# cvg/nicer-slam

Hardware: AMD Instinct MI355X
Metric: rays/sec (fwd+bwd), one tracking iteration (higher is better)
Workload: dtype f32; 1 GPU; Replica room0 tracking iteration, 1024 rays x 128 samples (+640 sampler evaluations/ray), single MI355X, fp32 [BASELINE configs[1]]; rays_per_gpu=1024, samples_per_ray=128, sampler_evals_per_ray=640, global_rays=1024, engine=fused, param_grads=False, hip_graph=True, driver=KernelTracker, python_gc=off inside the timed regions (as timeit), ray_chunks=1, cache_prewarm_steps=100, cache_prewarm_batches=disjoint from the warm-up and timed batches, parallelism=single, rccl_ranks=0, full=False

## Files before the change

nicer_slam_amd/csrc/colour_fwd_body.inc:

```
    desync_simd_partners();
    const int lane = threadIdx.x & 63;
    const int h = lane >> 5;
    const uint32_t tile = blockIdx.x * 4 + (threadIdx.x >> 6);
    if (tile * 32 >= a.src.P) return;
    const bool wave_live = true;
    uint32_t pid = tile * 32 + (lane & 31);
    const bool live = pid < a.src.P;
    if (!live) pid = a.src.P - 1;
    const uint32_t q = point_of(a.src, pid);
    float x[3], z, dir[3];
    uint32_t ray;
    load_point(a.src, q, x, ray, z);
#pragma unroll
    for (int d = 0; d < 3; ++d) dir[d] = a.src.rays_d[ray * 3 + d];
    float in[COL_IN_STEPS];
    colour_inputs(a, geom, tile, q, lane, h, x, dir, in, false, wave_live);
    f32x16 a1[2], a2[2];
    float rgb[3];
    uint32_t masks[2] = {0u, 0u};
    colour_mlp<Seq, false>(nullptr, a.wp, lane, h, in, a1, a2, rgb, a.save ? masks : nullptr);
    if (live && h == 0) {
#pragma unroll
        for (int j = 0; j < 3; ++j) a.rgb[(size_t)q * 3 + j] = rgb[j];
    }
    if (a.save) {
        float* ext = save_ext(a.save, a.src.P, tile);
        ext[lane] = __uint_as_float(masks[0]);
        ext[64 + lane] = __uint_as_float(masks[1]);
        if (h == 0) {
#pragma unroll
            for (int j = 0; j < 3; ++j) ext[128 + 32 * j + (lane & 31)] = rgb[j];
        }
    }
```

nicer_slam_amd/csrc/render_colour.hip:

```cpp
#include <cstdlib>
#include "sdf_net.hpp"

namespace nsa {

constexpr int CL = 16, CC = 2;

struct ColPack {
    static constexpr int kHH = a_block_floats(2, HS);
    static constexpr int kW0 = 0;
    static constexpr int kB0 = kW0 + a_block_floats(2, COL_IN_STEPS);
    static constexpr int kW1 = kB0 + 64;
    static constexpr int kB1 = kW1 + kHH;
    static constexpr int kW2V = kB1 + 64;
    static constexpr int kB2 = kW2V + 3 * 64;
    static constexpr int kW1T = kB2 + 64;
    static constexpr int kW0T = kW1T + kHH;
    static constexpr int kTotal = kW0T + a_block_floats(5, HS);
};

constexpr int kColStage = 7680;
template <bool BWD>
struct ColOps {
    static constexpr int n = BWD ? 6 : 3;
    __host__ __device__ static constexpr StageOp op(int i) {
        return i == 0 ? StageOp{ColPack::kW0, 2, 9, 0, 5} : i == 1 ? StageOp{ColPack::kW0, 2, 9, 5, 4}
             : i == 2 ? StageOp{ColPack::kW1, 2, 4, 0, 4} : i == 3 ? StageOp{ColPack::kW1T, 2, 4, 0, 4}
             : i == 4 ? StageOp{ColPack::kW0T, 5, 4, 0, 2} : StageOp{ColPack::kW0T, 5, 4, 2, 2};
    }
};

template <bool MAP>
struct ColBwdOps {
    static constexpr int n = MAP ? 6 : 3;
    static constexpr int kRev = MAP ? 3 : 0;
    __host__ __device__ static constexpr StageOp op(int i) { return ColOps<true>::op(MAP ? i : i + 3); }
};

constexpr int kSaveTile = 4096, kSaveExt = 256;
__device__ __forceinline__ float* save_ext(float* save, uint32_t P, uint32_t tile) {
    return save + (size_t)((P + 31) / 32) * kSaveTile + (size_t)tile * kSaveExt;
}

__device__ __forceinline__ uint32_t relu_mask(const f32x16 (&a)[2]) {
    uint32_t m = 0;
#pragma unroll
    for (int t = 0; t < 2; ++t)
#pragma unroll
        for (int r = 0; r < 16; ++r) m |= a[t][r] > 0.0f ? (1u << (16 * t + r)) : 0u;
    return m;
}

struct ColourArgs {
    PointSrc src;
    const float* table;
    const float* wp;
    float divide_factor;
    const float* grad;
    const float* feat;
    float* rgb;
    float* save;
    int save_no_features;
    const float* g_rgb;
    float* g_feat;
    float* g_grad;
    float* g_x;
    float* g_dir;
    int grid_grad;
    float* g_table;
    float* emit;
    uint32_t emit_ld;
};

enum : int { CE_IN = 0, CE_H1 = 130, CE_H2 = 194, CE_AB1 = 258, CE_AB2 = 322, CE_OB = 386, CE_ROWS = 389 };

struct ColEmitter {
    float* base;
    uint32_t ld;
    bool live;
    __device__ __forceinline__ void slot(int region, int s, int h, float v) const {
        base[(size_t)(region + 2 * s + h) * ld] = live ? v : 0.0f;
    }
    __device__ __forceinline__ void hid(int region, int q, int h, float v) const {
        const int f = 32 * (q >> 4) + (q & 3) + 8 * ((q & 15) >> 2) + 4 * h;
        base[(size_t)(region + f) * ld] = live ? v : 0.0f;
    }
};

__device__ __forceinline__ void colour_level_out(const float (&v)[8][CC], const float (&w)[3], const float (&dw)[3], float scale,
                                                 bool inside, int jl, float (&in)[COL_IN_STEPS], float* sv, bool sv_features = true) {
    float f[CC];
    blend<3, CC>(v, w, f);
#pragma unroll
    for (int c = 0; c < CC; ++c) in[49 + jl * CC + c] = inside ? f[c] : 0.0f;
    if (sv) {
        if (sv_features) {
#pragma unroll
            for (int c = 0; c < CC; ++c) sv[(jl * CC + c) * 64] = in[49 + jl * CC + c];
        }
#pragma unroll
        for (int gd = 0; gd < 3; ++gd) {
            float jr[CC];
            jacobian_row<3, CC>(v, w, dw, scale, gd, jr);
#pragma unroll
            for (int c = 0; c < CC; ++c) sv[(16 + (jl * 3 + gd) * CC + c) * 64] = inside ? jr[c] : 0.0f;
        }
    }
}

__device__ __forceinline__ void colour_inputs(const ColourArgs& a, const GridGeom16& geom, uint32_t tile, uint32_t q, int lane,
                                              int h, const float (&x)[3], const float (&dir)[3], float (&in)[COL_IN_STEPS],
                                              bool from_save, bool wave_live) {
    const float* fsrc = a.feat + (size_t)tile * 32 * 64 + lane;
#pragma unroll
    for (int q = 0; q < HS; ++q) in[q] = fsrc[q * 64];
    float gr[3];
#pragma unroll
    for (int d = 0; d < 3; ++d) gr[d] = a.grad[(size_t)q * 3 + d];
    in[32] = h ? x[1] : x[0];
    in[33] = h ? dir[0] : x[2];
    in[34] = h ? dir[2] : dir[1];
    in[35] = h ? gr[1] : gr[0];
    in[36] = h ? 0.0f : gr[2];
#pragma unroll
    for (int j = 0; j < 6; ++j) {
        const int g0 = 2 * j, g1 = 2 * j + 1;
        const float da = h ? dir[g1 % 3] : dir[g0 % 3];
        const float sc = h ? (float)(1 << (g1 / 3)) : (float)(1 << (g0 / 3));
        sincos_f(da * sc, in[37 + 2 * j], in[38 + 2 * j]);
    }
    if (from_save) {
        const float* sv = a.save + (size_t)tile * 64 * 64 + lane;
#pragma unroll
        for (int q = 0; q < 16; ++q) in[49 + q] = sv[q * 64];
        return;
    }
    float u[3];
#pragma unroll
    for (int d = 0; d < 3; ++d) u[d] = to_unit(x[d], a.divide_factor);
    float* sv = (a.save && wave_live) ? a.save + (size_t)tile * 64 * 64 + lane : nullptr;
#pragma unroll
    for (int jl = 0; jl < CL / 2; ++jl) {
        const LevelGeom lg = geom.lv[2 * jl + h];
        uint32_t cell[3];
        float w[3], dw[3];
        const bool inside = locate<3>(u, lg.scale, cell, w, dw);
        float v[8][CC];
        gather_corners<3, CC>(a.table, lg, cell, v);
        colour_level_out(v, w, dw, lg.scale, inside, jl, in, sv, !a.save_no_features);
    }
}

template <class Seq, bool STAGED>
__device__ __forceinline__ void colour_mlp(float* stage, const float* __restrict__ wp, int lane, int h,
                                           const float (&in)[COL_IN_STEPS], f32x16 (&a1)[2], f32x16 (&a2)[2], float (&rgb)[3],
                                           uint32_t* masks = nullptr) {
    load_vec<2>(wp + ColPack::kB0, h, a1);
    if (STAGED) {
        const float m_in = abs_max<COL_IN_STEPS>(in);
        gemm_staged_part<Seq, kColStage, COL_IN_STEPS, 2, 0, 5, true, false>(stage, wp, 0, lane, in, a1, &m_in);
        gemm_staged_part<Seq, kColStage, COL_IN_STEPS, 2, 5, 4, false, true>(stage, wp, 1, lane, in, a1, &m_in);
    } else {
        gemm_op<COL_IN_STEPS, 2>(wp + ColPack::kW0, lane, in, a1);
    }
    const float m_h1 = acc_abs_max<2>(a1);
    float h1[HS];
#pragma unroll
    for (int t = 0; t < 2; ++t)
#pragma unroll
        for (int r = 0; r < 16; ++r) h1[16 * t + r] = relu_f(a1[t][r]);
    if (masks) masks[0] = relu_mask(a1);
    load_vec<2>(wp + ColPack::kB1, h, a2);
    if (STAGED) gemm_staged_part<Seq, kColStage, HS, 2, 0, 4>(stage, wp, 2, lane, h1, a2, &m_h1);
    else        gemm_op<HS, 2>(wp + ColPack::kW1, lane, h1, a2, &m_h1);
    if (masks) masks[1] = relu_mask(a2);
#pragma unroll
    for (int j = 0; j < 3; ++j) {
        f32x16 wv[2];
        load_vec<2>(wp + ColPack::kW2V + 64 * j, h, wv);
        float part = 0.0f;
#pragma unroll
        for (int t = 0; t < 2; ++t)
#pragma unroll
            for (int r = 0; r < 16; ++r) part = fmaf(relu_f(a2[t][r]), wv[t][r], part);
        const float o = xhalf_sum(part) + wp[ColPack::kB2 + j];
        rgb[j] = 1.0f / (1.0f + expf(-o));
    }
}

#ifndef NSA_OCC_COL_FWD
#define NSA_OCC_COL_FWD 4
#endif
__global__ __launch_bounds__(256, NSA_OCC_COL_FWD) void k_colour_fwd(ColourArgs a, GridGeom16 geom) {
    using Seq = ColOps<false>;
#include "colour_fwd_body.inc"
}

#ifdef NSA_X_TS
static __device__ unsigned long long* g_ts_c = nullptr;
#define CTS_BEGIN const unsigned long long ts_start = ts_now(); unsigned long long ts_prev = ts_start; \
    if ((threadIdx.x & 63) == 0) for (int i = 0; i < 16; ++i) nsa_ts_lds[threadIdx.x >> 6][i] = 0;
#define CTS_MARK(slot) { const unsigned long long t_ = ts_now(); ts_add(slot, t_ - ts_prev); ts_prev = t_; }
#define CTS_END { ts_add(15, ts_now() - ts_start); if (g_ts_c && (threadIdx.x & 63) == 0) { \
    unsigned long long* o_ = g_ts_c + ((size_t)blockIdx.x * (blockDim.x >> 6) + (threadIdx.x >> 6)) * 16; \
    for (int i = 0; i < 16; ++i) o_[i] = nsa_ts_lds[threadIdx.x >> 6][i]; } }
#else
#define CTS_BEGIN
#define CTS_MARK(slot)
#define CTS_END
#endif
template <bool MAP>
__global__ __launch_bounds__(256, 2) void k_colour_bwd(ColourArgs a, GridGeom16 geom) {
    using Seq = ColBwdOps<MAP>;
    __shared__ __attribute__((aligned(16))) float stage[2 * kColStage];
    CTS_BEGIN
#define NSA_BODY_NW 4
#include "colour_bwd_body.inc"
#undef NSA_BODY_NW
    CTS_MARK(11)
    CTS_END
}

}

#define NSA_SDFNET_AS_HEADER
#include "render_sdfnet.hip"
#undef NSA_SDFNET_AS_HEADER

namespace nsa {

#define NSA_CC_NW 4
#define NSA_BODY_NW NSA_CC_NW
__global__ __launch_bounds__(64 * NSA_CC_NW, 2) void k_colour_coarse_bwd(ColourArgs ca, GridGeom16 cgeom, SdfNetArgs sa, GridGeom16 sgeom) {
    __shared__ __attribute__((aligned(16))) float stage[2 * kStageFloats];
    static_assert(kStageFloats >= kColStage, "the colour phase stages its parts in the SDF kernel's buffers");
    float ho_fb[HS], ho_n[3], ho_gx[3];
#define NSA_BODY_HANDOFF
    {
        constexpr bool MAP = false;
        using Seq = ColBwdOps<false>;
        const ColourArgs& a = ca;
        const GridGeom16& geom = cgeom;
#include "colour_bwd_body.inc"
    }
    __syncthreads();
    {
        constexpr int L = 4, C = 8, NH = 1;
        constexpr bool MAP = false;
        using P = SdfPack<NH>;
        using Seq = SdfOps<NH, true>;
        const SdfNetArgs& a = sa;
        const GridGeom16& geom = sgeom;
#include "sdfnet_bwd_body.inc"
    }
#undef NSA_BODY_HANDOFF
}
#undef NSA_BODY_NW

}

#define NSA_COMPOSITE_AS_HEADER
#include "render_composite.hip"
#undef NSA_COMPOSITE_AS_HEADER

namespace nsa {

__global__ __launch_bounds__(256, NSA_OCC_COL_FWD) void k_colour_fwd_track(ColourArgs ca, GridGeom16 cgeom, CompositeArgs ta,
                                                                            const float* __restrict__ gt, float* __restrict__ ray_loss,
                                                                            float inv_n) {
    {
        using Seq = ColOps<false>;
        const ColourArgs& a = ca;
        const GridGeom16& geom = cgeom;
#include "colour_fwd_body.inc"
    }
    __syncthreads();
    if ((threadIdx.x >> 6) == 0) {
        const CompositeArgs& a = ta;
        const int lane = threadIdx.x & 63;
        const uint32_t ray = blockIdx.x;
#include "composite_track_body.inc"
    }
}

__global__ __launch_bounds__(256, NSA_OCC_COL_FWD) void k_colour_fwd_composite(ColourArgs ca, GridGeom16 cgeom, CompositeArgs ta) {
    {
        using Seq = ColOps<false>;
        const ColourArgs& a = ca;
        const GridGeom16& geom = cgeom;
#include "colour_fwd_body.inc"
    }
    __syncthreads();
    if ((threadIdx.x >> 6) == 0) {
        const CompositeArgs& a = ta;
        const int lane = threadIdx.x & 63;
        const uint32_t ray = blockIdx.x;
#include "composite_fwd_body.inc"
    }
}

}

#if defined(NSA_X_TS) && NSA_PIECES != 1
extern "C" int nsa_debug_set_ts_colour(unsigned long long* p) {
    return hipMemcpyToSymbol(HIP_SYMBOL(nsa::g_ts_c), &p, sizeof(p)) == hipSuccess ? 0 : 3;
}
#endif

#ifndef NSA_ENTRY
#define NSA_ENTRY(x) x
#endif
#include "bf16_entries.hpp"

extern "C" {

static int colour_common(const nsa_points_t* pts, const nsa_grid_t* grid, nsa::ColourArgs* a, nsa::GridGeom16* geom) {
    using namespace nsa;
    if (!pts || !grid) return NSA_EBADARG;
    if (pts->points || !pts->rays_o || !pts->rays_d || !pts->z_vals || pts->S == 0) return NSA_EBADARG;
    if (!(grid->L == 16 && grid->C == 2)) return NSA_EUNSUPPORTED_NET;
    if (int rc = make_grid_geom16(grid->offsets_host, grid->L, grid->S, grid->H, geom, grid->C)) return rc;
    a->src = PointSrc{pts->rays_o, pts->rays_d, pts->z_vals, nullptr, pts->P, pts->S, pts->order};
    a->table = grid->table;
    a->divide_factor = grid->divide_factor;
    return NSA_OK;
}

int NSA_ENTRY(nsa_colour_forward)(const nsa_points_t* pts, const nsa_grid_t* grid, const float* packed, const float* grad,
                       const float* feat_hl, float* rgb, float* save, nsa_stream_t stream) {
#if NSA_PIECES != 1
    if (grid && grid->precision == 1) return nsa_colour_forward_bf16(pts, grid, packed, grad, feat_hl, rgb, save, stream);
#endif
    using namespace nsa;
    if (!packed || !grad || !feat_hl || !rgb) return NSA_EBADARG;
    ColourArgs a{};
    GridGeom16 geom;
    if (int rc = colour_common(pts, grid, &a, &geom)) return rc;
    if (pts->P == 0) return NSA_OK;
    a.wp = packed; a.grad = grad; a.feat = feat_hl; a.rgb = rgb; a.save = save;
    const uint32_t tiles = (pts->P + 31) / 32;
    launch_begin();
    hipLaunchKernelGGL(k_colour_fwd, dim3((tiles + 3) / 4), dim3(256), 0, (hipStream_t)stream, a, geom);
    return launch_end();
}

int NSA_ENTRY(nsa_colour_forward_composite)(const nsa_points_t* pts, const nsa_grid_t* grid, const float* packed, const float* grad,
                                 const float* feat_hl, float* rgb, float* save, const float* sdf, const float* voxels,
                                 uint32_t voxel_res, float* weights, float* rgb_values, float* depth, float* nmap, float* entropy,
                                 nsa_stream_t stream) {
#if NSA_PIECES != 1
    if (grid && grid->precision == 1)
        return nsa_colour_forward_composite_bf16(pts, grid, packed, grad, feat_hl, rgb, save, sdf, voxels, voxel_res, weights, rgb_values,
                                                 depth, nmap, entropy, stream);
#endif
    using namespace nsa;
    if (!packed || !grad || !feat_hl || !rgb || !sdf || !voxels || !weights || !rgb_values || !depth || !nmap || !entropy)
        return NSA_EBADARG;
    ColourArgs a{};
    GridGeom16 geom;
    if (int rc = colour_common(pts, grid, &a, &geom)) return rc;
    if (pts->P == 0) return NSA_OK;
    if (pts->points || pts->order || pts->S != 128 || pts->P % 128 != 0) return NSA_EBADARG;
    a.wp = packed; a.grad = grad; a.feat = feat_hl; a.rgb = rgb; a.save = save;
    CompositeArgs t{};
    t.rays_o = pts->rays_o; t.rays_d = pts->rays_d; t.z_vals = pts->z_vals; t.sdf = sdf; t.rgb = rgb; t.grad = grad; t.voxels = voxels;
    t.voxel_res = voxel_res; t.R = pts->P / 128; t.S = 128;
    t.weights = weights; t.rgb_values = rgb_values; t.depth = depth; t.nmap = nmap; t.entropy = entropy;
    launch_begin();
    hipLaunchKernelGGL(k_colour_fwd_composite, dim3(pts->P / 128), dim3(256), 0, (hipStream_t)stream, a, geom, t);
    return launch_end();
}

int NSA_ENTRY(nsa_colour_forward_track)(const nsa_points_t* pts, const nsa_grid_t* grid, const float* packed, const float* grad,
                             const float* feat_hl, float* rgb, float* save, const float* sdf, const float* voxels, uint32_t voxel_res,
                             const float* gt, uint32_t n_total, float* rgb_values, float* ray_loss, float* g_sdf, float* g_rgb,
                             float* g_grad, nsa_stream_t stream) {
#if NSA_PIECES != 1
    if (grid && grid->precision == 1)
        return nsa_colour_forward_track_bf16(pts, grid, packed, grad, feat_hl, rgb, save, sdf, voxels, voxel_res, gt, n_total, rgb_values,
                                             ray_loss, g_sdf, g_rgb, g_grad, stream);
#endif
    using namespace nsa;
    if (!packed || !grad || !feat_hl || !rgb || !sdf || !voxels || !gt || !rgb_values || !ray_loss || !g_sdf || !g_rgb || !g_grad)
        return NSA_EBADARG;
    ColourArgs a{};
    GridGeom16 geom;
    if (int rc = colour_common(pts, grid, &a, &geom)) return rc;
    if (pts->P == 0) return NSA_OK;
    if (pts->points || pts->order || pts->S != 128 || pts->P % 128 != 0 || n_total < pts->P / 128) return NSA_EBADARG;
    a.wp = packed; a.grad = grad; a.feat = feat_hl; a.rgb = rgb; a.save = save;
#ifndef NSA_X_SAVE_FEATURES
    a.save_no_features = 1;
#endif
    CompositeArgs t{};
    t.rays_o = pts->rays_o; t.rays_d = pts->rays_d; t.z_vals = pts->z_vals; t.sdf = sdf; t.rgb = rgb; t.voxels = voxels;
    t.voxel_res = voxel_res; t.R = pts->P / 128; t.S = 128;
    t.rgb_values = rgb_values; t.g_sdf = g_sdf; t.g_rgb = g_rgb; t.g_grad = g_grad;
    launch_begin();
    hipLaunchKernelGGL(k_colour_fwd_track, dim3(pts->P / 128), dim3(256), 0, (hipStream_t)stream, a, geom, t, gt, ray_loss,
                       1.0f / (float)(3 * (uint64_t)n_total));
    return launch_end();
}

int NSA_ENTRY(nsa_colour_backward)(const nsa_points_t* pts, const nsa_grid_t* grid, const float* packed, const float* grad,
                        const float* feat_hl, const float* save, const float* g_rgb, int grid_grad, float* g_feat_hl,
                        float* g_grad, float* g_x, float* g_dir, nsa_stream_t stream) {
#if NSA_PIECES != 1
    if (grid && grid->precision == 1) return nsa_colour_backward_bf16(pts, grid, packed, grad, feat_hl, save, g_rgb, grid_grad, g_feat_hl, g_grad, g_x, g_dir, stream);
#endif
    using namespace nsa;
    if (!packed || !grad || !feat_hl || !save || !g_rgb || !g_feat_hl || !g_grad || !g_x || !g_dir) return NSA_EBADARG;
    ColourArgs a{};
    GridGeom16 geom;
    if (int rc = colour_common(pts, grid, &a, &geom)) return rc;
    if (pts->P == 0) return NSA_OK;
    a.wp = packed; a.grad = grad; a.feat = feat_hl; a.save = const_cast<float*>(save); a.g_rgb = g_rgb;
    a.g_feat = g_feat_hl; a.g_grad = g_grad; a.g_x = g_x; a.g_dir = g_dir; a.grid_grad = grid_grad;
    const uint32_t tiles = (pts->P + 31) / 32;
    launch_begin();
    hipLaunchKernelGGL(k_colour_bwd<false>, dim3((tiles + 3) / 4), dim3(256), 0, (hipStream_t)stream, a, geom);
    return launch_end();
}

int NSA_ENTRY(nsa_colour_coarse_backward)(const nsa_points_t* pts, const nsa_grid_t* grid, const float* packed, const float* grad,
                               const float* feat_hl, const float* save, const float* g_rgb, int grid_grad, float* g_feat_hl,
                               float* g_grad, float* g_x, float* g_dir, const nsa_grid_t* coarse, const float* packed_coarse,
                               const float* g_sdf, nsa_stream_t stream) {
#if NSA_PIECES != 1
    if (grid && coarse && grid->precision == 1 && coarse->precision == 1)
        return nsa_colour_coarse_backward_bf16(pts, grid, packed, grad, feat_hl, save, g_rgb, grid_grad, g_feat_hl, g_grad, g_x, g_dir, coarse,
                                               packed_coarse, g_sdf, stream);
#endif
    using namespace nsa;
    if (!packed || !grad || !feat_hl || !save || !g_rgb || !g_feat_hl || !g_grad || !g_x || !g_dir || !coarse || !packed_coarse)
        return NSA_EBADARG;
    if (grid->precision != coarse->precision) return NSA_EBADARG;
    if (coarse->tile == 16 || !(coarse->L == 4 && coarse->C == 8 && coarse->n_hidden == 1)) return NSA_EUNSUPPORTED_NET;
    ColourArgs a{};
    GridGeom16 geom, sgeom;
    if (int rc = colour_common(pts, grid, &a, &geom)) return rc;
    if (pts->P == 0) return NSA_OK;
    if (int rc = make_grid_geom16(coarse->offsets_host, coarse->L, coarse->S, coarse->H, &sgeom, coarse->C)) return rc;
    a.wp = packed; a.grad = grad; a.feat = feat_hl; a.save = const_cast<float*>(save); a.g_rgb = g_rgb;
    a.g_feat = g_feat_hl; a.g_grad = g_grad; a.g_x = g_x; a.g_dir = g_dir; a.grid_grad = grid_grad;
    SdfNetArgs sa{};
    sa.src = a.src;
    sa.table = coarse->table; sa.wp = packed_coarse; sa.divide_factor = coarse->divide_factor; sa.accumulate = 1;
    sa.g_sdf = g_sdf; sa.g_feat = g_feat_hl; sa.g_grad = g_grad; sa.g_x = g_x;
    const uint32_t tiles = (pts->P + 31) / 32;
    launch_begin();
    hipLaunchKernelGGL(k_colour_coarse_bwd, dim3((tiles + NSA_CC_NW - 1) / NSA_CC_NW), dim3(64 * NSA_CC_NW), 0, (hipStream_t)stream, a, geom, sa, sgeom);
    return launch_end();
}

int NSA_ENTRY(nsa_colour_backward_params)(const nsa_points_t* pts, const nsa_grid_t* grid, const float* packed, const float* grad,
                               const float* feat_hl, const float* save, const float* g_rgb, int grid_grad,
                               float* g_feat_hl, float* g_grad, float* g_x, float* g_dir, float* g_table, float* emit,
                               uint32_t emit_ld, nsa_stream_t stream) {
#if NSA_PIECES != 1
    if (grid && grid->precision == 1) return nsa_colour_backward_params_bf16(pts, grid, packed, grad, feat_hl, save, g_rgb, grid_grad, g_feat_hl, g_grad, g_x, g_dir, g_table, emit, emit_ld, stream);
#endif
    using namespace nsa;
    if (!packed || !grad || !feat_hl || !save || !g_rgb || !g_feat_hl || !g_grad || !g_x || !g_dir) return NSA_EBADARG;
    if (!g_table && !emit) return NSA_EBADARG;
    ColourArgs a{};
    GridGeom16 geom;
    if (int rc = colour_common(pts, grid, &a, &geom)) return rc;
    if (pts->P == 0) return NSA_OK;
    if (emit && emit_ld < ((pts->P + 31) / 32) * 32) return NSA_EBADARG;
    a.wp = packed; a.grad = grad; a.feat = feat_hl; a.save = const_cast<float*>(save); a.g_rgb = g_rgb;
    a.g_feat = g_feat_hl; a.g_grad = g_grad; a.g_x = g_x; a.g_dir = g_dir; a.grid_grad = grid_grad;
    a.g_table = g_table; a.emit = emit; a.emit_ld = emit_ld;
    const uint32_t tiles = (pts->P + 31) / 32;
    launch_begin();
    hipLaunchKernelGGL(k_colour_bwd<true>, dim3((tiles + 3) / 4), dim3(256), 0, (hipStream_t)stream, a, geom);
    return launch_end();
}

int NSA_ENTRY(nsa_colour_emit_rows)(void) { return nsa::CE_ROWS; }

}
```

nicer_slam_amd/csrc/render_composite.hip:

```cpp
#include "sdf_net.hpp"

namespace nsa {

constexpr int MAX_PER = 4;

__device__ __forceinline__ float beta_at(const float* __restrict__ voxels, uint32_t res, const float (&x)[3]) {
    const bool outside = fabsf(x[0]) > 0.99f || fabsf(x[1]) > 0.99f || fabsf(x[2]) > 0.99f;
    float count = 0.0f;
    if (!outside) {
        int idx[3];
#pragma unroll
        for (int k = 0; k < 3; ++k) {
            const int v = (int)((x[k] + 1.0f) / 2.0f * (float)res);
            idx[k] = v < 0 ? 0 : (v >= (int)res ? (int)res - 1 : v);
        }
        count = voxels[((size_t)idx[0] * res + idx[1]) * res + idx[2]];
    }
    return 0.01207724805f * expf(-0.0116544676f * 0.0001f * count * 5.37538f) + 0.0023639156f;
}

__device__ __forceinline__ float wave_sum(float v) {
#pragma unroll
    for (int off = 32; off > 0; off >>= 1) v += __shfl_xor(v, off);
    return v;
}

__device__ __forceinline__ float wave_excl(float v, int lane, float& total) {
    float incl = v;
#pragma unroll
    for (int off = 1; off < 64; off <<= 1) {
        const float n = __shfl_up(incl, off);
        if (lane >= off) incl += n;
    }
    total = __shfl(incl, 63);
    const float prev = __shfl_up(incl, 1);
    return lane == 0 ? 0.0f : prev;
}

struct CompositeArgs {
    const float* rays_o;
    const float* rays_d;
    const float* z_vals;
    const float* sdf;
    const float* rgb;
    const float* grad;
    const float* voxels;
    uint32_t voxel_res, R, S;
    float* weights;
    float* rgb_values;
    float* depth;
    float* nmap;
    float* entropy;
    const float* g_rgbv;
    const float* g_depth;
    const float* g_nmap;
    const float* g_ent;
    const float* g_w;
    float* g_sdf;
    float* g_rgb;
    float* g_grad;
};

struct Sample {
    float z, dist, sdf, beta, sigma, en, w, T;
};

__device__ __forceinline__ int ray_forward(const CompositeArgs& a, uint32_t ray, int lane, uint32_t per, Sample (&sm)[MAX_PER]) {
    const uint32_t S = a.S;
    float o[3], d[3];
#pragma unroll
    for (int k = 0; k < 3; ++k) { o[k] = a.rays_o[ray * 3 + k]; d[k] = a.rays_d[ray * 3 + k]; }
    const float* zr = a.z_vals + (size_t)ray * S;
    const float* sr = a.sdf + (size_t)ray * S;
    const uint32_t i0 = lane * per;
    float esum = 0.0f;
    int n = 0;
#pragma unroll
    for (int k = 0; k < MAX_PER; ++k) {
        const uint32_t i = i0 + k;
        if ((uint32_t)k < per && i < S) {
            Sample& s = sm[k];
            s.z = zr[i];
            s.dist = i + 1 < S ? zr[i + 1] - s.z : 1e10f;
            s.sdf = sr[i];
            float x[3];
#pragma unroll
            for (int c = 0; c < 3; ++c) x[c] = o[c] + mul_rn(s.z, d[c]);
            s.beta = beta_at(a.voxels, a.voxel_res, x);
            const float sg = s.sdf > 0.0f ? 1.0f : (s.sdf < 0.0f ? -1.0f : 0.0f);
            s.sigma = (1.0f / s.beta) * (0.5f + 0.5f * sg * expm1f(-fabsf(s.sdf) / s.beta));
            s.en = s.dist * s.sigma;
            esum += s.en;
            n = k + 1;
        }
    }
    float tot;
    float run = wave_excl(esum, lane, tot);
#pragma unroll
    for (int k = 0; k < MAX_PER; ++k) {
        if (k < n) {
            Sample& s = sm[k];
            s.T = expf(-run);
            s.w = (1.0f - expf(-s.en)) * s.T;
            run += s.en;
        }
    }
    return n;
}

#ifndef NSA_COMPOSITE_AS_HEADER
__global__ __launch_bounds__(256) void k_composite_fwd(CompositeArgs a) {
    const int lane = threadIdx.x & 63;
    const uint32_t ray = blockIdx.x * 4 + (threadIdx.x >> 6);
    if (ray >= a.R) return;
#include "composite_fwd_body.inc"
}

__global__ __launch_bounds__(256) void k_composite_bwd(CompositeArgs a) {
    const int lane = threadIdx.x & 63;
    const uint32_t ray = blockIdx.x * 4 + (threadIdx.x >> 6);
    if (ray >= a.R) return;
    const uint32_t S = a.S, per = (S + 63) / 64;
    Sample sm[MAX_PER];
    const int n = ray_forward(a, ray, lane, per, sm);
    float grv[3] = {0, 0, 0}, gnm[3] = {0, 0, 0};
#pragma unroll
    for (int c = 0; c < 3; ++c) {
        if (a.g_rgbv) grv[c] = a.g_rgbv[ray * 3 + c];
        if (a.g_nmap) gnm[c] = a.g_nmap[ray * 3 + c];
    }
    const float gdep = a.g_depth ? a.g_depth[ray] : 0.0f;
    const float gent = a.g_ent ? a.g_ent[ray] : 0.0f;
    float A = 0.0f, B = 0.0f;
#pragma unroll
    for (int k = 0; k < MAX_PER; ++k)
        if (k < n) { A = fmaf(sm[k].w, sm[k].z, A); B += sm[k].w; }
    A = wave_sum(A);
    B = wave_sum(B) + 1e-8f;
    float wbar[MAX_PER], ww = 0.0f;
#pragma unroll
    for (int k = 0; k < MAX_PER; ++k) {
        wbar[k] = 0.0f;
        if (k < n) {
            const size_t i = (size_t)ray * S + lane * per + k;
            const Sample& s = sm[k];
            float g[3], c3[3];
#pragma unroll
            for (int c = 0; c < 3; ++c) { c3[c] = a.rgb[i * 3 + c]; g[c] = a.grad[i * 3 + c]; }
            const float nrm = sqrtf(g[0] * g[0] + g[1] * g[1] + g[2] * g[2]);
            const float inv = 1.0f / (nrm + 1e-6f);
            float wb = grv[0] * c3[0] + grv[1] * c3[1] + grv[2] * c3[2];
            wb += gdep * (s.z * B - A) / (B * B);
            wb += (gnm[0] * g[0] + gnm[1] * g[1] + gnm[2] * g[2]) * inv;
            wb += gent * (-logf(s.w + 1e-4f) - s.w / (s.w + 1e-4f));
            if (a.g_w) wb += a.g_w[i];
            wbar[k] = wb;
            ww += wb * s.w;
            const float gdot = (g[0] * gnm[0] + g[1] * gnm[1] + g[2] * gnm[2]) * s.w;
            const float k2 = nrm > 0.0f ? gdot * inv * inv / nrm : 0.0f;
#pragma unroll
            for (int c = 0; c < 3; ++c) {
                a.g_rgb[i * 3 + c] = s.w * grv[c];
                a.g_grad[i * 3 + c] = s.w * gnm[c] * inv - g[c] * k2;
            }
        }
    }
    float later = ww;
#pragma unroll
    for (int off = 1; off < 64; off <<= 1) {
        const float n2 = __shfl_down(later, off);
        if (lane + off < 64) later += n2;
    }
    float suffix = __shfl_down(later, 1);
    if (lane == 63) suffix = 0.0f;
#pragma unroll
    for (int k = MAX_PER - 1; k >= 0; --k) {
        if (k < n) {
            const size_t i = (size_t)ray * S + lane * per + k;
            const Sample& s = sm[k];
            const float Tn = s.T * expf(-s.en);
            const float eb = wbar[k] * Tn - suffix;
            suffix += wbar[k] * s.w;
            const float sb = eb * s.dist;
            const float sg = s.sdf > 0.0f ? 1.0f : (s.sdf < 0.0f ? -1.0f : 0.0f);
            const float em1 = expm1f(-fabsf(s.sdf) / s.beta) + 1.0f;
            const float dsig = -0.5f * sg * sg * em1 / (s.beta * s.beta);
            a.g_sdf[i] = sb * dsig;
        }
    }
}

__global__ __launch_bounds__(256) void k_composite_track(CompositeArgs a, const float* __restrict__ gt, float* __restrict__ ray_loss,
                                                         float inv_n) {
    const int lane = threadIdx.x & 63;
    const uint32_t ray = blockIdx.x * 4 + (threadIdx.x >> 6);
    if (ray >= a.R) return;
#include "composite_track_body.inc"
}

__global__ __launch_bounds__(256) void k_rays_bwd(const float* __restrict__ z_vals, const float* __restrict__ g_x,
                                                  const float* __restrict__ g_dir, float* __restrict__ g_o,
                                                  float* __restrict__ g_d, uint32_t R, uint32_t S) {
    const int lane = threadIdx.x & 63;
    const uint32_t ray = blockIdx.x * 4 + (threadIdx.x >> 6);
    if (ray >= R) return;
    float acc[6] = {0, 0, 0, 0, 0, 0};
    for (uint32_t i = lane; i < S; i += 64) {
        const size_t p = (size_t)ray * S + i;
        const float z = z_vals[p];
#pragma unroll
        for (int c = 0; c < 3; ++c) {
            const float gx = g_x[p * 3 + c];
            acc[c] += gx;
            acc[3 + c] += z * gx + (g_dir ? g_dir[p * 3 + c] : 0.0f);
        }
    }
#pragma unroll
    for (int q = 0; q < 6; ++q) acc[q] = wave_sum(acc[q]);
    if (lane == 0) {
#pragma unroll
        for (int c = 0; c < 3; ++c) { g_o[ray * 3 + c] = acc[c]; g_d[ray * 3 + c] = acc[3 + c]; }
    }
}

#endif

}

#ifndef NSA_COMPOSITE_AS_HEADER
extern "C" {

int nsa_composite_forward(const float* rays_o, const float* rays_d, const float* z_vals, const float* sdf, const float* rgb,
                          const float* grad, const float* voxels, uint32_t voxel_res, uint32_t R, uint32_t S, float* weights,
                          float* rgb_values, float* depth, float* nmap, float* entropy, nsa_stream_t stream) {
    using namespace nsa;
    if (R == 0) return NSA_OK;
    if (!rays_o || !rays_d || !z_vals || !sdf || !rgb || !grad || !voxels || !weights || !rgb_values || !depth || !nmap ||
        !entropy || S == 0 || S > 64 * MAX_PER)
        return NSA_EBADARG;
    CompositeArgs a{};
    a.rays_o = rays_o; a.rays_d = rays_d; a.z_vals = z_vals; a.sdf = sdf; a.rgb = rgb; a.grad = grad; a.voxels = voxels;
    a.voxel_res = voxel_res; a.R = R; a.S = S;
    a.weights = weights; a.rgb_values = rgb_values; a.depth = depth; a.nmap = nmap; a.entropy = entropy;
    launch_begin();
    hipLaunchKernelGGL(k_composite_fwd, dim3((R + 3) / 4), dim3(256), 0, (hipStream_t)stream, a);
    return launch_end();
}

int nsa_composite_backward(const float* rays_o, const float* rays_d, const float* z_vals, const float* sdf, const float* rgb,
                           const float* grad, const float* voxels, uint32_t voxel_res, uint32_t R, uint32_t S,
                           const float* g_rgb_values, const float* g_depth, const float* g_nmap, const float* g_entropy,
                           const float* g_weights, float* g_sdf, float* g_rgb, float* g_grad, nsa_stream_t stream) {
    using namespace nsa;
    if (R == 0) return NSA_OK;
    if (!rays_o || !rays_d || !z_vals || !sdf || !rgb || !grad || !voxels || !g_sdf || !g_rgb || !g_grad || S == 0 ||
        S > 64 * MAX_PER)
        return NSA_EBADARG;
    CompositeArgs a{};
    a.rays_o = rays_o; a.rays_d = rays_d; a.z_vals = z_vals; a.sdf = sdf; a.rgb = rgb; a.grad = grad; a.voxels = voxels;
    a.voxel_res = voxel_res; a.R = R; a.S = S;
    a.g_rgbv = g_rgb_values; a.g_depth = g_depth; a.g_nmap = g_nmap; a.g_ent = g_entropy; a.g_w = g_weights;
    a.g_sdf = g_sdf; a.g_rgb = g_rgb; a.g_grad = g_grad;
    launch_begin();
    hipLaunchKernelGGL(k_composite_bwd, dim3((R + 3) / 4), dim3(256), 0, (hipStream_t)stream, a);
    return launch_end();
}

int nsa_composite_track(const float* rays_o, const float* rays_d, const float* z_vals, const float* sdf, const float* rgb,
                        const float* voxels, uint32_t voxel_res, uint32_t R, uint32_t S, const float* gt, uint32_t n_total,
                        float* rgb_values, float* ray_loss, float* g_sdf, float* g_rgb, float* g_grad, nsa_stream_t stream) {
    using namespace nsa;
    if (R == 0) return NSA_OK;
    if (!rays_o || !rays_d || !z_vals || !sdf || !rgb || !voxels || !gt || !rgb_values || !ray_loss || !g_sdf || !g_rgb ||
        !g_grad || S == 0 || S > 64 * MAX_PER || n_total < R)
        return NSA_EBADARG;
    CompositeArgs a{};
    a.rays_o = rays_o; a.rays_d = rays_d; a.z_vals = z_vals; a.sdf = sdf; a.rgb = rgb; a.voxels = voxels;
    a.voxel_res = voxel_res; a.R = R; a.S = S;
    a.rgb_values = rgb_values; a.g_sdf = g_sdf; a.g_rgb = g_rgb; a.g_grad = g_grad;
    launch_begin();
    hipLaunchKernelGGL(k_composite_track, dim3((R + 3) / 4), dim3(256), 0, (hipStream_t)stream, a, gt, ray_loss,
                       1.0f / (float)(3 * (uint64_t)n_total));
    return launch_end();
}

int nsa_rays_backward(const float* z_vals, const float* g_x, const float* g_dir, uint32_t R, uint32_t S, float* g_rays_o,
                      float* g_rays_d, nsa_stream_t stream) {
    using namespace nsa;
    if (R == 0) return NSA_OK;
    if (!z_vals || !g_x || !g_rays_o || !g_rays_d || S == 0) return NSA_EBADARG;
    launch_begin();
    hipLaunchKernelGGL(k_rays_bwd, dim3((R + 3) / 4), dim3(256), 0, (hipStream_t)stream, z_vals, g_x, g_dir, g_rays_o,
                       g_rays_d, R, S);
    return launch_end();
}

}
#endif
```

Before: 2.049 million rays/s.

## Overlap composite weight computation with colour MLP in fused track kernel

The fused colour-forward and track kernel now starts the first wave's composite work early. It issues the ray loads (origin, direction, z, sdf, target) at the head of the colour body, then gathers voxel counts and computes transmittance weights into shared memory while the MLP runs. Colour outputs are staged in LDS so the tail reads them without a global round-trip, and zeroing of g_grad moves into the per-point colour path. The tail is specialised for 128 samples per ray. This hides composite latency behind the MLP, at the cost of more registers and LDS in the first wave, which may reduce occupancy.

```diff
diff --git a/nicer_slam_amd/csrc/colour_fwd_body.inc b/nicer_slam_amd/csrc/colour_fwd_body.inc
--- a/nicer_slam_amd/csrc/colour_fwd_body.inc
+++ b/nicer_slam_amd/csrc/colour_fwd_body.inc
@@ -1,9 +1,14 @@
+#ifndef NSA_COLFWD_HOOK
+#define NSA_COLFWD_HOOK(at)
+#define NSA_COLFWD_HOOK_IS_EMPTY
+#endif
     desync_simd_partners();
     const int lane = threadIdx.x & 63;
     const int h = lane >> 5;
     const uint32_t tile = blockIdx.x * 4 + (threadIdx.x >> 6);
     if (tile * 32 >= a.src.P) return;
     const bool wave_live = true;
+    NSA_COLFWD_HOOK(HEAD)
     uint32_t pid = tile * 32 + (lane & 31);
     const bool live = pid < a.src.P;
     if (!live) pid = a.src.P - 1;
@@ -13,12 +18,15 @@
     load_point(a.src, q, x, ray, z);
 #pragma unroll
     for (int d = 0; d < 3; ++d) dir[d] = a.src.rays_d[ray * 3 + d];
+    NSA_COLFWD_HOOK(POINT)
     float in[COL_IN_STEPS];
     colour_inputs(a, geom, tile, q, lane, h, x, dir, in, false, wave_live);
+    NSA_COLFWD_HOOK(INPUTS)
     f32x16 a1[2], a2[2];
     float rgb[3];
     uint32_t masks[2] = {0u, 0u};
     colour_mlp<Seq, false>(nullptr, a.wp, lane, h, in, a1, a2, rgb, a.save ? masks : nullptr);
+    NSA_COLFWD_HOOK(OUT)
     if (live && h == 0) {
 #pragma unroll
         for (int j = 0; j < 3; ++j) a.rgb[(size_t)q * 3 + j] = rgb[j];
@@ -32,3 +40,7 @@
             for (int j = 0; j < 3; ++j) ext[128 + 32 * j + (lane & 31)] = rgb[j];
         }
     }
+#ifdef NSA_COLFWD_HOOK_IS_EMPTY
+#undef NSA_COLFWD_HOOK_IS_EMPTY
+#undef NSA_COLFWD_HOOK
+#endif
diff --git a/nicer_slam_amd/csrc/composite_track_tail128.inc b/nicer_slam_amd/csrc/composite_track_tail128.inc
--- /dev/null
+++ b/nicer_slam_amd/csrc/composite_track_tail128.inc
@@ -0,0 +1,66 @@
+    constexpr uint32_t S = kRayS, per = kRayPer;
+    float c3[kRayPer][3], sw[kRayPer];
+#pragma unroll
+    for (int k = 0; k < kRayPer; ++k) {
+        const uint32_t i = lane * per + k;
+        sw[k] = rs.w[i];
+#ifdef NSA_X_TAIL_RGB_GLOBAL
+#pragma unroll
+        for (int c = 0; c < 3; ++c) c3[k][c] = a.rgb[((size_t)ray * S + i) * 3 + c];
+#else
+#pragma unroll
+        for (int c = 0; c < 3; ++c) c3[k][c] = rs.rgb[i * 3 + c];
+#endif
+    }
+    float acc[3] = {0, 0, 0};
+#pragma unroll
+    for (int k = 0; k < kRayPer; ++k) {
+#pragma unroll
+        for (int c = 0; c < 3; ++c) acc[c] = fmaf(sw[k], c3[k][c], acc[c]);
+    }
+    float grv[3], l = 0.0f;
+#pragma unroll
+    for (int c = 0; c < 3; ++c) {
+        acc[c] = wave_sum(acc[c]);
+        const float d = acc[c] - tgt[c];
+        l += fabsf(d);
+        grv[c] = d > 0.0f ? inv_n : (d < 0.0f ? -inv_n : 0.0f);
+    }
+    if (lane == 0) {
+#pragma unroll
+        for (int c = 0; c < 3; ++c) a.rgb_values[ray * 3 + c] = acc[c];
+        ray_loss[ray] = l;
+    }
+    float wbar[kRayPer], ww = 0.0f;
+#pragma unroll
+    for (int k = 0; k < kRayPer; ++k) {
+        const size_t i = (size_t)ray * S + lane * per + k;
+        const float w = sw[k];
+        const float wb = grv[0] * c3[k][0] + grv[1] * c3[k][1] + grv[2] * c3[k][2];
+        wbar[k] = wb;
+        ww += wb * w;
+#pragma unroll
+        for (int c = 0; c < 3; ++c) {
+            a.g_rgb[i * 3 + c] = w * grv[c];
+#ifdef NSA_X_TAIL_ZEROS
+            a.g_grad[i * 3 + c] = 0.0f;
+#endif
+        }
+    }
+    float later = ww;
+#pragma unroll
+    for (int off = 1; off < 64; off <<= 1) {
+        const float n2 = __shfl_down(later, off);
+        if (lane + off < 64) later += n2;
+    }
+    float suffix = __shfl_down(later, 1);
+    if (lane == 63) suffix = 0.0f;
+#pragma unroll
+    for (int k = kRayPer - 1; k >= 0; --k) {
+        const uint32_t j = lane * per + k;
+        const size_t i = (size_t)ray * S + j;
+        const float eb = wbar[k] * rs.Tn[j] - suffix;
+        suffix += wbar[k] * sw[k];
+        const float sb = eb * rs.dist[j];
+        a.g_sdf[i] = sb * rs.dsig[j];
+    }
diff --git a/nicer_slam_amd/csrc/render_colour.hip b/nicer_slam_amd/csrc/render_colour.hip
--- a/nicer_slam_amd/csrc/render_colour.hip
+++ b/nicer_slam_amd/csrc/render_colour.hip
@@ -267,18 +267,43 @@
 __global__ __launch_bounds__(256, NSA_OCC_COL_FWD) void k_colour_fwd_track(ColourArgs ca, GridGeom16 cgeom, CompositeArgs ta,
                                                                             const float* __restrict__ gt, float* __restrict__ ray_loss,
                                                                             float inv_n) {
+    __shared__ Ray128Lds rs;
+    Ray128Head rh;
+    const bool first_wave = (threadIdx.x >> 6) == 0;
+#define NSA_TRACK_HEAD if (first_wave) ray128_request(ta, gt, blockIdx.x, lane, rh);
+#ifndef NSA_X_TAIL_ZEROS
+#define NSA_TRACK_POINT                                                                          \
+    if (first_wave) { ray128_gather(ta, lane, rh); ray128_weights(lane, rh, rs); }           \
+    if (h == 0) {                                                                                \
+        _Pragma("unroll") for (int c = 0; c < 3; ++c) ta.g_grad[(size_t)q * 3 + c] = 0.0f;       \
+    }
+#else
+#define NSA_TRACK_POINT if (first_wave) { ray128_gather(ta, lane, rh); ray128_weights(lane, rh, rs); }
+#endif
+#define NSA_TRACK_INPUTS
+#ifndef NSA_X_TAIL_RGB_GLOBAL
+#define NSA_TRACK_OUT                                                                                                     \
+    if (h == 0) {                                                                                                         \
+        _Pragma("unroll") for (int j = 0; j < 3; ++j) rs.rgb[((threadIdx.x >> 6) * 32 + (lane & 31)) * 3 + j] = rgb[j];   \
+    }
+#else
+#define NSA_TRACK_OUT
+#endif
+#define NSA_COLFWD_HOOK(at) NSA_TRACK_##at
     {
         using Seq = ColOps<false>;
         const ColourArgs& a = ca;
         const GridGeom16& geom = cgeom;
 #include "colour_fwd_body.inc"
     }
+#undef NSA_COLFWD_HOOK
     __syncthreads();
-    if ((threadIdx.x >> 6) == 0) {
+    if (first_wave) {
         const CompositeArgs& a = ta;
-        const int lane = threadIdx.x & 63;
+        const int lane = __lane_id();
         const uint32_t ray = blockIdx.x;
-#include "composite_track_body.inc"
+        const float (&tgt)[3] = rh.tgt;
+#include "composite_track_tail128.inc"
     }
 }
 
diff --git a/nicer_slam_amd/csrc/render_composite.hip b/nicer_slam_amd/csrc/render_composite.hip
--- a/nicer_slam_amd/csrc/render_composite.hip
+++ b/nicer_slam_amd/csrc/render_composite.hip
@@ -4,7 +4,7 @@
 
 constexpr int MAX_PER = 4;
 
-__device__ __forceinline__ float beta_at(const float* __restrict__ voxels, uint32_t res, const float (&x)[3]) {
+__device__ __forceinline__ float visit_count(const float* __restrict__ voxels, uint32_t res, const float (&x)[3]) {
     const bool outside = fabsf(x[0]) > 0.99f || fabsf(x[1]) > 0.99f || fabsf(x[2]) > 0.99f;
     float count = 0.0f;
     if (!outside) {
@@ -16,7 +16,15 @@
         }
         count = voxels[((size_t)idx[0] * res + idx[1]) * res + idx[2]];
     }
+    return count;
+}
+
+__device__ __forceinline__ float beta_of_count(float count) {
     return 0.01207724805f * expf(-0.0116544676f * 0.0001f * count * 5.37538f) + 0.0023639156f;
+}
+
+__device__ __forceinline__ float beta_at(const float* __restrict__ voxels, uint32_t res, const float (&x)[3]) {
+    return beta_of_count(visit_count(voxels, res, x));
 }
 
 __device__ __forceinline__ float wave_sum(float v) {
@@ -108,6 +116,70 @@
     return n;
 }
 
+constexpr int kRayS = 128, kRayPer = 2;
+
+struct Ray128Lds {
+    float dist[kRayS], w[kRayS], Tn[kRayS], dsig[kRayS];
+    float rgb[kRayS * 3];
+};
+
+struct Ray128Head {
+    float o[3], d[3], tgt[3], z[kRayPer + 1], sdf[kRayPer], dist[kRayPer], count[kRayPer];
+};
+
+__device__ __forceinline__ void ray128_request(const CompositeArgs& a, const float* __restrict__ gt, uint32_t ray, int lane,
+                                               Ray128Head& r) {
+#pragma unroll
+    for (int k = 0; k < 3; ++k) { r.o[k] = a.rays_o[ray * 3 + k]; r.d[k] = a.rays_d[ray * 3 + k]; r.tgt[k] = gt[ray * 3 + k]; }
+    const float* zr = a.z_vals + (size_t)ray * kRayS;
+    const float* sr = a.sdf + (size_t)ray * kRayS;
+    const uint32_t i0 = lane * kRayPer;
+#pragma unroll
+    for (int k = 0; k <= kRayPer; ++k) r.z[k] = i0 + k < (uint32_t)kRayS ? zr[i0 + k] : 0.0f;
+#pragma unroll
+    for (int k = 0; k < kRayPer; ++k) r.sdf[k] = sr[i0 + k];
+}
+
+__device__ __forceinline__ void ray128_gather(const CompositeArgs& a, int lane, Ray128Head& r) {
+#pragma unroll
+    for (int k = 0; k < kRayPer; ++k) {
+        const uint32_t i = lane * kRayPer + k;
+        const float z = r.z[k];
+        r.dist[k] = i + 1 < (uint32_t)kRayS ? r.z[k + 1] - z : 1e10f;
+        float x[3];
+#pragma unroll
+        for (int c = 0; c < 3; ++c) x[c] = r.o[c] + mul_rn(z, r.d[c]);
+        r.count[k] = visit_count(a.voxels, a.voxel_res, x);
+    }
+}
+
+__device__ __forceinline__ void ray128_weights(int lane, const Ray128Head& r, Ray128Lds& s) {
+    float en[kRayPer], esum = 0.0f;
+#pragma unroll
+    for (int k = 0; k < kRayPer; ++k) {
+        const uint32_t i = lane * kRayPer + k;
+        const float sdf = r.sdf[k], dist = r.dist[k];
+        const float beta = beta_of_count(r.count[k]);
+        const float sg = sdf > 0.0f ? 1.0f : (sdf < 0.0f ? -1.0f : 0.0f);
+        const float sigma = (1.0f / beta) * (0.5f + 0.5f * sg * expm1f(-fabsf(sdf) / beta));
+        en[k] = dist * sigma;
+        esum += en[k];
+        const float em1 = expm1f(-fabsf(sdf) / beta) + 1.0f;
+        s.dsig[i] = -0.5f * sg * sg * em1 / (beta * beta);
+        s.dist[i] = dist;
+    }
+    float tot;
+    float run = wave_excl(esum, lane, tot);
+#pragma unroll
+    for (int k = 0; k < kRayPer; ++k) {
+        const uint32_t i = lane * kRayPer + k;
+        const float T = expf(-run);
+        s.w[i] = (1.0f - expf(-en[k])) * T;
+        s.Tn[i] = T * expf(-en[k]);
+        run += en[k];
+    }
+}
+
 #ifndef NSA_COMPOSITE_AS_HEADER
 __global__ __launch_bounds__(256) void k_composite_fwd(CompositeArgs a) {
     const int lane = threadIdx.x & 63;
```

Result: slower. 2.024 million rays/s (-1.2%).
